# kepingbi/ProdSearch

Measured on AMD Instinct MI355X. Metric: train (u,q,i,neg) tuples/sec at bs=384, 20 neg, d=128, higher is better.
Workload: dtype f32 (fp32 MFMA and VALU; wide products, the fused per-replica kernels and grouped weight gradients as fp32-grade bf16x3 products: exact 3-way bf16 split of both fp32 operands, 6 of the 9 cross products as bf16 MFMAs per step, fp32 accumulation); 1 GPU; item_transformer d=128 1 layer 8 heads ff=512 uprev=20 bs=384/GPU 20 neg Q=8 W=1 P=18357 V=32387 dropout=0.10 (BASELINE configs[1]); global_batch=384, parallelism=dp1, step=sample+fwd+bwd+clip/Adam via nn.Module API (trainer.py:74-78), replicas_per_row=21

## Files before the change

### include/prodsearch_hip.h

```cpp
#ifndef PRODSEARCH_HIP_H
#define PRODSEARCH_HIP_H

#include <stddef.h>
#include <stdint.h>

#ifdef __cplusplus
extern "C" {
#endif

#define PS_MAX_LAYERS 8
#define PS_OK 0
#define PS_ERR_ARG 1
#define PS_ERR_HIP 2

typedef void* ps_stream_t;

enum { PS_MODEL_TEM = 0, PS_MODEL_QEM = 1,
       PS_MODEL_AEM = 2,
       PS_MODEL_ZAM = 3 };
enum { PS_QENC_FS = 0, PS_QENC_AVG = 1 };

typedef struct PsTemDesc {
  int32_t B;
  int32_t K;
// ... 45 lines not shown

typedef struct PsTemBatch {
  const int64_t *query_word_idxs;
  const int64_t *target_prod_idxs;
  const int64_t *u_item_idxs;
  const int64_t *pos_iword_idxs;
  const int64_t *neg_item_idxs;
  const int64_t *neg_word_idxs;
  const int64_t *candi_prod_idxs;
} PsTemBatch;

typedef struct PsTemWsLayout {
  int64_t total_floats;
  int32_t R;
  int32_t S;
  int64_t qmean, query_emb, x;
  int64_t kp, vp, qp, attn, ctx;
  int64_t y1, ln1, a1, h1, y2, enc;
  int64_t item_scores, word_scores, loss_parts;
  int64_t denc, dx;
} PsTemWsLayout;

const char* ps_version(void);
const char* ps_last_error(void);
const char* ps_arith_info(void);
int ps_set_fuse_bwd_min(int rows);
int ps_set_item_scatter_fused(int on);
int ps_item_scatter_fused_taken(void);
typedef struct PsEncPath {
  int32_t n_layers;
  int32_t attn[PS_MAX_LAYERS];
  int32_t rowlist, fwd_fuse_last, fold_score;
  int32_t bwd_fuse_last, item_scatter, wg3_main, wg3_last, wgrad_early, q_folded, listed, presum, dx_fused;
  int32_t wf_key_split;
} PsEncPath;
int ps_tem_plan(const PsTemDesc* desc, const PsTemTensors* params, int32_t has_valid, PsEncPath* out);
int ps_enc_path_taken(int32_t backward, PsEncPath* out);
int ps_set_side_mode(int mode);
int ps_side_values_in_use(void);
void ps_side_abort(void);
void ps_debug_fail_fork(int nth);
int ps_set_deterministic(int on);
int ps_gemm_x3_config(int mode, int force_shape);
int ps_gemm_f32_weight(const float* A, int lda, const float* W, int tb, float* C, int ldc, int M, int N, int K,
                       const float* bias, float alpha, ps_stream_t stream);

int ps_tem_workspace_layout(const PsTemDesc* desc, PsTemWsLayout* out);

int ps_tem_forward(const PsTemDesc* desc, const PsTemTensors* params, const PsTemBatch* batch,
                   float* workspace, float* loss3, float* loss_acc, ps_stream_t stream);
int ps_tem_forward_sampled(const PsTemDesc* desc, const PsTemTensors* params, const PsTemBatch* batch,
                           const float* alias_prob, const int32_t* alias_idx, int64_t* neg_item_out, int64_t* neg_word_out,
                           float* workspace, float* loss3, float* loss_acc, ps_stream_t stream);

int ps_tem_backward(const PsTemDesc* desc, const PsTemTensors* params, const PsTemBatch* batch,
                    float* workspace, const PsTemTensors* grads, float loss_scale,
                    const float* loss_scale_dev ,
                    ps_stream_t stream);

int ps_gather_score(const PsTemDesc* desc, const PsTemTensors* params, const PsTemBatch* batch,
                    float* workspace, ps_stream_t stream);

int ps_tem_score(const PsTemDesc* desc, const PsTemTensors* params, const PsTemBatch* batch,
                 float* workspace, float* scores, ps_stream_t stream);

int ps_sample_negatives(const PsTemDesc* desc, const float* alias_prob, const int32_t* alias_idx,
                        int64_t* neg_item_idxs, int64_t* neg_word_idxs, ps_stream_t stream);
int ps_build_alias_host(const double* dist_host, int64_t n, float* prob_host, int32_t* alias_host);

typedef struct PsAdamHyper {
  float lr;
  float beta1, beta2;
  float eps;
  float weight_decay;
  float max_grad_norm;
  int32_t noam;
  int32_t warmup_steps;
  float grad_scale;
  int32_t zero_grads;
  int32_t method;
  int32_t pad_;
} PsAdamHyper;

int64_t ps_adam_plan_bytes(int32_t n_tensors, const int64_t* numel_host);
int ps_adam_plan_write_host(int32_t n_tensors, float* const* p, float* const* g, float* const* m,
                            float* const* v, const int64_t* numel_host, void* plan_host);
int32_t ps_adam_plan_chunks_host(const void* plan_host);
int ps_clip_adam_dense(const void* plan_dev, int32_t n_chunks, const PsAdamHyper* hyper,
                       int64_t* state_dev, float* gnorm_out_dev ,
                       ps_stream_t stream);

int ps_adam_sumsq(const void* plan_dev, int32_t n_chunks, const PsAdamHyper* hyper, int64_t* state_dev,
                  float* out_sumsq_dev, ps_stream_t stream);
int ps_adam_update_ext(const void* plan_dev, int32_t n_chunks, const PsAdamHyper* hyper, int64_t* state_dev,
                       const float* total_sumsq_dev, float* gnorm_out_dev, ps_stream_t stream);

int ps_sum_slices(const float* recv, int32_t world, int64_t n, float* out, float* zero, int64_t zero_n, ps_stream_t stream);

int ps_zero_floats(float* p, int64_t n, ps_stream_t stream);

int ps_graph_replay_enabled(void);
int ps_tem_staged_batch(const PsTemDesc* desc, float* workspace, PsTemBatch* out);
int ps_tem_forward_step(const PsTemDesc* desc, const PsTemTensors* params, const PsTemBatch* batch,
                        const float* sampler_prob, const int32_t* sampler_alias, float* workspace, float* loss3,
                        float* loss_acc, ps_stream_t stream);
int ps_tem_backward_step(const PsTemDesc* desc, const PsTemTensors* params, float* workspace, const PsTemTensors* grads,
                         float loss_scale, float* zero_ptr, int64_t zero_floats, ps_stream_t stream);

int ps_tem_encode(const PsTemDesc* desc, const PsTemTensors* params, const PsTemBatch* batch, float* workspace,
                  float* enc_out , ps_stream_t stream);
int64_t ps_rank_scratch_bytes(int32_t B, int64_t n_rows, int32_t d, int32_t topk);
int ps_rank_all(const float* q, int32_t B, int32_t d, const float* table, int64_t n_rows, const float* bias,
                const int64_t* target, int32_t topk, int64_t* top_idx, float* top_score, int32_t* rank,
                void* scratch, int64_t scratch_bytes, ps_stream_t stream);
int ps_rank_shard(const float* q, int32_t B, int32_t d, const float* table, int64_t n_rows, const float* bias,
                  const int64_t* target, const float* target_score, int64_t id_mul, int64_t id_add, int32_t topk,
                  int64_t* top_idx, float* top_score, int32_t* ahead, void* scratch, int64_t scratch_bytes, ps_stream_t stream);

typedef struct PsIdxList { const int64_t* idx; int64_t n; } PsIdxList;

int64_t ps_coalesce_ws_bytes(int64_t n_rows);
int ps_coalesce_rows(const PsIdxList* lists_host, int32_t n_lists, int64_t n_rows, int64_t pad_row, void* ws_dev,
                     int64_t* rows_out_dev, int64_t cap, int32_t* count_out_dev, ps_stream_t stream);
int ps_gather_rows(const float* table_dev, int32_t d, const int64_t* rows_dev, const int32_t* count_dev, int64_t cap,
                   float* values_out_dev, ps_stream_t stream);
int ps_scatter_rows(float* table_dev, int32_t d, const int64_t* rows_dev, const int32_t* count_dev, int64_t cap,
                    const float* values_dev, ps_stream_t stream);
int ps_zero_rows(float* table_dev, int32_t d, const int64_t* rows_dev, const int32_t* count_dev, int64_t cap,
                 ps_stream_t stream);
const int32_t* ps_coalesce_bad_flag(void* ws_dev, int64_t n_rows);

int ps_pack_rows(const float* grad_dev, int32_t d, const int64_t* rows_dev, const int32_t* count_dev, int64_t cap,
                 int64_t* msg_rows_dev, float* msg_vals_dev, ps_stream_t stream);
int ps_merge_rows(const int64_t* all_rows_dev, const float* all_vals_dev, int32_t world, int64_t cap, int32_t d,
                  float* grad_dev, const int64_t* union_rows_dev, const int32_t* union_count_dev, int64_t union_cap,
                  ps_stream_t stream);

typedef struct PsRowTable {
  float* p; float* g; float* m; float* v;
  const int64_t* rows;
  const int32_t* count;
  int64_t cap;
  int32_t d;
  int32_t pad_;
} PsRowTable;

int64_t ps_adam_rowsparse_state_floats(int32_t n_chunks, const PsRowTable* tables_host, int32_t n_tables);
int ps_clip_adam_rowsparse(const void* plan_dev, int32_t n_chunks, const PsRowTable* tables_host, int32_t n_tables,
                           const PsAdamHyper* hyper, int64_t* state_dev, float* gnorm_out_dev, ps_stream_t stream);

int ps_rowsparse_catchup(const PsRowTable* tables_host, int32_t n_tables, int32_t* const* last_dev, const int64_t* n_rows_host,
                         const PsAdamHyper* hyper, const int64_t* state_dev, int32_t advance, int32_t all_rows,
                         ps_stream_t stream);

int ps_shard_bucket(const int64_t* rows_dev, const int32_t* count_dev, int32_t world, int64_t capp, int64_t* send_ids_dev,
                    int32_t* slot_of_dev, int32_t* bad_dev, ps_stream_t stream);
int ps_shard_remap(const int64_t* idx_dev, int64_t n, int64_t pad_in, const int64_t* rows_dev, const int32_t* count_dev,
                   const int32_t* slot_of_dev, int64_t pad_out, int64_t* out_dev, int32_t* bad_dev, ps_stream_t stream);
int ps_rowsparse_sumsq(const void* plan_dev, int32_t n_chunks, const PsRowTable* tables_host, int32_t n_tables, int32_t n_shared,
                       const PsAdamHyper* hyper, int64_t* state_dev, float* sums_dev, ps_stream_t stream);
int ps_rowsparse_update_ext(const void* plan_dev, int32_t n_chunks, const PsRowTable* tables_host, int32_t n_tables,
                            const PsAdamHyper* hyper, int64_t* state_dev, const float* sums_dev, float* gnorm_out_dev,
                            ps_stream_t stream);

enum { PS_RENC_PV = 0, PS_RENC_PVC = 1,
       PS_RENC_FS = 2,
// ... 103 lines not shown
```

### prodsearch_amd/_lib.py

```python
import ctypes as C
import os

from . import build as _build

PS_MAX_LAYERS = 8
PS_MODEL_TEM, PS_MODEL_QEM, PS_MODEL_AEM, PS_MODEL_ZAM = 0, 1, 2, 3
PS_QENC_FS, PS_QENC_AVG = 0, 1

_f32p = C.POINTER(C.c_float)
_i64p = C.POINTER(C.c_int64)


class PsTemDesc(C.Structure):
    _fields_ = [(n, C.c_int32) for n in ('B', 'K', 'L', 'Q', 'W', 'C', 'd', 'H', 'F', 'n_layers')] + \
               [('product_size', C.c_int64), ('vocab_size', C.c_int64)] + \
               [(n, C.c_int32) for n in ('model', 'query_encoder', 'use_pos_emb', 'use_item_pos',
                                         'bias_product', 'pos_weight', 'sep_prod_emb', 'training')] + \
               [('dropout', C.c_float), ('seed', C.c_uint64), ('step', C.c_uint64)]


LAYER_FIELDS = ('wk', 'bk', 'wv', 'bv', 'wq', 'bq', 'wo', 'bo', 'w1', 'b1', 'w2', 'b2',
                'ff_ln_g', 'ff_ln_b', 'ln_g', 'ln_b')
TOP_FIELDS = ('product_emb', 'hist_product_emb', 'word_emb', 'product_bias', 'word_bias',
              'fs_w', 'fs_b', 'pe', 'final_ln_g', 'final_ln_b')
# ... 40 lines not shown
class PsRowTable(C.Structure):
    _fields_ = [('p', C.c_void_p), ('g', C.c_void_p), ('m', C.c_void_p), ('v', C.c_void_p),
                ('rows', C.c_void_p), ('count', C.c_void_p), ('cap', C.c_int64), ('d', C.c_int32),
                ('pad_', C.c_int32)]


class PsRtmDesc(C.Structure):
    _fields_ = [(n, C.c_int32) for n in ('B', 'K', 'R', 'Q', 'W', 'WL', 'C', 'd', 'H', 'F', 'n_layers')] + \
               [('vocab_size', C.c_int64), ('review_count', C.c_int64)] + \
               [(n, C.c_int32) for n in ('review_encoder', 'query_encoder', 'use_pos_emb', 'use_seg_emb',
                                         'pos_weight', 'train_pv', 'training')] + \
               [('dropout', C.c_float), ('corrupt_rate', C.c_float), ('seed', C.c_uint64), ('step', C.c_uint64)] + \
               [('use_user_emb', C.c_int32), ('use_item_emb', C.c_int32), ('user_size', C.c_int64),
                ('product_size', C.c_int64)]


RTM_TOP_FIELDS = ('word_emb', 'review_emb', 'seg_emb', 'fs_w', 'fs_b', 'pe', 'final_ln_g', 'final_ln_b',
                  'wo_w', 'wo_b', 'user_emb', 'product_emb', 'rev_fs_w', 'rev_fs_b')
RTM_BATCH_FIELDS = ('query_word_idxs', 'pos_prod_ridxs', 'pos_seg_idxs', 'pos_prod_rword_idxs',
                    'pos_prod_rword_masks', 'neg_prod_ridxs', 'neg_seg_idxs', 'neg_prod_rword_idxs',
                    'pos_prod_rword_idxs_pvc', 'neg_prod_rword_idxs_pvc', 'neg_word_idxs',
                    'candi_prod_ridxs', 'candi_seg_idxs', 'review_embeddings', 'pos_user_idxs', 'neg_user_idxs',
                    'pos_item_idxs', 'neg_item_idxs', 'candi_seq_user_idxs', 'candi_seq_item_idxs', 'neg_prod_rword_masks')


class PsRtmTensors(C.Structure):
    _fields_ = [(n, C.c_void_p) for n in RTM_TOP_FIELDS] + [('layer', PsLayerTensors * PS_MAX_LAYERS)]


class PsRtmBatch(C.Structure):
    _fields_ = [(n, C.c_void_p) for n in RTM_BATCH_FIELDS]


class PsRtmWsLayout(C.Structure):
    _fields_ = [('total_floats', C.c_int64)] + [(n, C.c_int32) for n in ('Bseq', 'S', 'J', 'pad_')] + \
               [(n, C.c_int64) for n in ('query_emb', 'valid', 'x', 'vec', 'cnt', 'enc', 'scores', 'weight',
                                         'pv_scores', 'dx')]


PS_RENC_PV, PS_RENC_PVC, PS_RENC_FS, PS_RENC_AVG = 0, 1, 2, 3

SYMBOLS = {
    'ps_version': (C.c_char_p, []),
    'ps_last_error': (C.c_char_p, []),
    'ps_arith_info': (C.c_char_p, []),
    'ps_set_fuse_bwd_min': (C.c_int, [C.c_int]),
    'ps_set_item_scatter_fused': (C.c_int, [C.c_int]),
    'ps_item_scatter_fused_taken': (C.c_int, []),
    'ps_tem_plan': (C.c_int, [C.POINTER(PsTemDesc), C.POINTER(PsTemTensors), C.c_int32, C.POINTER(PsEncPath)]),
    'ps_enc_path_taken': (C.c_int, [C.c_int32, C.POINTER(PsEncPath)]),
    'ps_set_side_mode': (C.c_int, [C.c_int]),
    'ps_side_values_in_use': (C.c_int, []),
    'ps_set_deterministic': (C.c_int, [C.c_int]),
    'ps_side_abort': (None, []),
    'ps_debug_fail_fork': (None, [C.c_int]),
    'ps_gemm_x3_config': (C.c_int, [C.c_int, C.c_int]),
    'ps_gemm_f32_weight': (C.c_int, [C.c_void_p, C.c_int, C.c_void_p, C.c_int, C.c_void_p, C.c_int, C.c_int, C.c_int, C.c_int,
                                     C.c_void_p, C.c_float, C.c_void_p]),
    'ps_tem_workspace_layout': (C.c_int, [C.POINTER(PsTemDesc), C.POINTER(PsTemWsLayout)]),
    'ps_tem_forward': (C.c_int, [C.POINTER(PsTemDesc), C.POINTER(PsTemTensors), C.POINTER(PsTemBatch),
                                 C.c_void_p, C.c_void_p, C.c_void_p, C.c_void_p]),
    'ps_tem_forward_sampled': (C.c_int, [C.POINTER(PsTemDesc), C.POINTER(PsTemTensors), C.POINTER(PsTemBatch),
                                         C.c_void_p, C.c_void_p, C.c_void_p, C.c_void_p, C.c_void_p, C.c_void_p, C.c_void_p,
                                         C.c_void_p]),
    'ps_tem_backward': (C.c_int, [C.POINTER(PsTemDesc), C.POINTER(PsTemTensors), C.POINTER(PsTemBatch),
                                  C.c_void_p, C.POINTER(PsTemTensors), C.c_float, C.c_void_p, C.c_void_p]),
    'ps_gather_score': (C.c_int, [C.POINTER(PsTemDesc), C.POINTER(PsTemTensors), C.POINTER(PsTemBatch),
                                  C.c_void_p, C.c_void_p]),
    'ps_tem_score': (C.c_int, [C.POINTER(PsTemDesc), C.POINTER(PsTemTensors), C.POINTER(PsTemBatch),
                               C.c_void_p, C.c_void_p, C.c_void_p]),
    'ps_rtm_workspace_floats': (C.c_int, [C.POINTER(PsRtmDesc), C.c_int32, C.POINTER(C.c_int64)]),
    'ps_rtm_workspace_layout': (C.c_int, [C.POINTER(PsRtmDesc), C.c_int32, C.POINTER(PsRtmWsLayout)]),
    'ps_rtm_forward': (C.c_int, [C.POINTER(PsRtmDesc), C.POINTER(PsRtmTensors), C.POINTER(PsRtmBatch),
                                 C.c_void_p, C.c_void_p, C.c_void_p]),
    'ps_rtm_backward': (C.c_int, [C.POINTER(PsRtmDesc), C.POINTER(PsRtmTensors), C.POINTER(PsRtmBatch),
                                  C.c_void_p, C.POINTER(PsRtmTensors), C.c_float, C.c_void_p, C.c_void_p]),
    'ps_rtm_score': (C.c_int, [C.POINTER(PsRtmDesc), C.POINTER(PsRtmTensors), C.POINTER(PsRtmBatch),
                               C.c_void_p, C.c_void_p, C.c_void_p]),
    'ps_rtm_review_embeddings': (C.c_int, [C.POINTER(PsRtmDesc), C.POINTER(PsRtmTensors), C.c_void_p,
                                           C.c_void_p, C.c_void_p, C.c_void_p]),
    'ps_sample_negatives': (C.c_int, [C.POINTER(PsTemDesc), C.c_void_p, C.c_void_p, C.c_void_p,
                                      C.c_void_p, C.c_void_p]),
    'ps_build_alias_host': (C.c_int, [C.c_void_p, C.c_int64, C.c_void_p, C.c_void_p]),
    'ps_adam_plan_bytes': (C.c_int64, [C.c_int32, C.c_void_p]),
    'ps_adam_plan_write_host': (C.c_int, [C.c_int32, C.c_void_p, C.c_void_p, C.c_void_p, C.c_void_p,
                                          C.c_void_p, C.c_void_p]),
    'ps_adam_plan_chunks_host': (C.c_int32, [C.c_void_p]),
    'ps_clip_adam_dense': (C.c_int, [C.c_void_p, C.c_int32, C.POINTER(PsAdamHyper), C.c_void_p,
                                     C.c_void_p, C.c_void_p]),
    'ps_adam_sumsq': (C.c_int, [C.c_void_p, C.c_int32, C.POINTER(PsAdamHyper), C.c_void_p, C.c_void_p, C.c_void_p]),
    'ps_adam_update_ext': (C.c_int, [C.c_void_p, C.c_int32, C.POINTER(PsAdamHyper), C.c_void_p, C.c_void_p, C.c_void_p,
                                     C.c_void_p]),
    'ps_dropout_mult_host': (C.c_float, [C.POINTER(PsTemDesc), C.c_uint32, C.c_uint32, C.c_uint32]),
    'ps_zero_floats': (C.c_int, [C.c_void_p, C.c_int64, C.c_void_p]),
    'ps_sum_slices': (C.c_int, [C.c_void_p, C.c_int32, C.c_int64, C.c_void_p, C.c_void_p, C.c_int64, C.c_void_p]),
    'ps_graph_replay_enabled': (C.c_int, []),
    'ps_tem_staged_batch': (C.c_int, [C.POINTER(PsTemDesc), C.c_void_p, C.POINTER(PsTemBatch)]),
    'ps_tem_forward_step': (C.c_int, [C.POINTER(PsTemDesc), C.POINTER(PsTemTensors), C.POINTER(PsTemBatch), C.c_void_p,
                                      C.c_void_p, C.c_void_p, C.c_void_p, C.c_void_p, C.c_void_p]),
    'ps_tem_backward_step': (C.c_int, [C.POINTER(PsTemDesc), C.POINTER(PsTemTensors), C.c_void_p, C.POINTER(PsTemTensors),
                                       C.c_float, C.c_void_p, C.c_int64, C.c_void_p]),
    'ps_tem_encode': (C.c_int, [C.POINTER(PsTemDesc), C.POINTER(PsTemTensors), C.POINTER(PsTemBatch),
                                C.c_void_p, C.c_void_p, C.c_void_p]),
    'ps_rank_scratch_bytes': (C.c_int64, [C.c_int32, C.c_int64, C.c_int32, C.c_int32]),
    'ps_rank_all': (C.c_int, [C.c_void_p, C.c_int32, C.c_int32, C.c_void_p, C.c_int64, C.c_void_p, C.c_void_p, C.c_int32,
                              C.c_void_p, C.c_void_p, C.c_void_p, C.c_void_p, C.c_int64, C.c_void_p]),
    'ps_rank_shard': (C.c_int, [C.c_void_p, C.c_int32, C.c_int32, C.c_void_p, C.c_int64, C.c_void_p, C.c_void_p, C.c_void_p,
                                C.c_int64, C.c_int64, C.c_int32, C.c_void_p, C.c_void_p, C.c_void_p, C.c_void_p, C.c_int64,
                                C.c_void_p]),
    'ps_coalesce_ws_bytes': (C.c_int64, [C.c_int64]),
    'ps_coalesce_rows': (C.c_int, [C.POINTER(PsIdxList), C.c_int32, C.c_int64, C.c_int64, C.c_void_p,
                                   C.c_void_p, C.c_int64, C.c_void_p, C.c_void_p]),
    'ps_gather_rows': (C.c_int, [C.c_void_p, C.c_int32, C.c_void_p, C.c_void_p, C.c_int64, C.c_void_p, C.c_void_p]),
    'ps_scatter_rows': (C.c_int, [C.c_void_p, C.c_int32, C.c_void_p, C.c_void_p, C.c_int64, C.c_void_p, C.c_void_p]),
    'ps_zero_rows': (C.c_int, [C.c_void_p, C.c_int32, C.c_void_p, C.c_void_p, C.c_int64, C.c_void_p]),
    'ps_coalesce_bad_flag': (C.c_void_p, [C.c_void_p, C.c_int64]),
    'ps_pack_rows': (C.c_int, [C.c_void_p, C.c_int32, C.c_void_p, C.c_void_p, C.c_int64, C.c_void_p, C.c_void_p,
                               C.c_void_p]),
    'ps_merge_rows': (C.c_int, [C.c_void_p, C.c_void_p, C.c_int32, C.c_int64, C.c_int32, C.c_void_p, C.c_void_p,
                                C.c_void_p, C.c_int64, C.c_void_p]),
    'ps_adam_rowsparse_state_floats': (C.c_int64, [C.c_int32, C.POINTER(PsRowTable), C.c_int32]),
    'ps_clip_adam_rowsparse': (C.c_int, [C.c_void_p, C.c_int32, C.POINTER(PsRowTable), C.c_int32,
                                         C.POINTER(PsAdamHyper), C.c_void_p, C.c_void_p, C.c_void_p]),
    'ps_shard_bucket': (C.c_int, [C.c_void_p, C.c_void_p, C.c_int32, C.c_int64, C.c_void_p, C.c_void_p, C.c_void_p, C.c_void_p]),
    'ps_shard_remap': (C.c_int, [C.c_void_p, C.c_int64, C.c_int64, C.c_void_p, C.c_void_p, C.c_void_p, C.c_int64, C.c_void_p,
                                 C.c_void_p, C.c_void_p]),
    'ps_rowsparse_sumsq': (C.c_int, [C.c_void_p, C.c_int32, C.POINTER(PsRowTable), C.c_int32, C.c_int32, C.POINTER(PsAdamHyper),
                                     C.c_void_p, C.c_void_p, C.c_void_p]),
    'ps_rowsparse_update_ext': (C.c_int, [C.c_void_p, C.c_int32, C.POINTER(PsRowTable), C.c_int32, C.POINTER(PsAdamHyper),
                                          C.c_void_p, C.c_void_p, C.c_void_p, C.c_void_p]),
    'ps_rowsparse_catchup': (C.c_int, [C.POINTER(PsRowTable), C.c_int32, C.POINTER(C.c_void_p), C.POINTER(C.c_int64),
                                       C.POINTER(PsAdamHyper), C.c_void_p, C.c_int32, C.c_int32, C.c_void_p]),
    'ps_ktimer_arm': (C.c_int, [C.c_char_p, C.c_int32]),
    'ps_ktimer_read': (C.c_int, [C.POINTER(C.c_double), C.POINTER(C.c_double), C.POINTER(C.c_int32)]),
    'ps_gemm_f32': (C.c_int, [C.c_void_p, C.c_int, C.c_int, C.c_void_p, C.c_int, C.c_int, C.c_void_p,
                              C.c_int, C.c_int, C.c_int, C.c_int, C.c_void_p, C.c_float, C.c_int,
                              C.c_void_p]),
}

class PsCorpusView(C.Structure):
    _fields_ = [(n, C.c_int64) for n in ('n_reviews', 'n_users', 'n_products', 'n_queries')] + \
               [(n, C.c_void_p) for n in ('review_u_p', 'u_seq_ptr', 'u_seq', 'train_review', 'review_loc',
                                          'pq_ptr', 'pq_idx', 'query_words')] + \
               [('Q', C.c_int32), ('pad_', C.c_int32)]


class PsCollateArgs(C.Structure):
    _fields_ = [('uprev_review_limit', C.c_int32), ('do_seq', C.c_int32), ('fix', C.c_int32), ('pad_', C.c_int32),
                ('prod_pad', C.c_int64)]


class PsTrainSlot(C.Structure):
    _fields_ = [(n, C.c_void_p) for n in ('query_words', 'target', 'u_items', 'pos_words', 'query_idx', 'user_idx', 'hist_len')]


class PsRtmCorpusView(C.Structure):
    _fields_ = [(n, C.c_int64) for n in ('n_reviews', 'n_users', 'n_products', 'n_queries')] + \
               [(n, C.c_void_p) for n in ('review_u_p', 'u_seq_ptr', 'u_seq', 'i_seq_ptr', 'i_seq', 'ut_seq_ptr', 'ut_seq',
                                          'it_seq_ptr', 'it_seq', 'loc_time', 'pq_ptr', 'pq_idx', 'query_words')] + \
               [('Q', C.c_int32), ('pad_', C.c_int32)]


class PsRtmCollateArgs(C.Structure):
    _fields_ = [('uprev_review_limit', C.c_int32), ('iprev_review_limit', C.c_int32), ('do_seq', C.c_int32),
                ('neg_per_pos', C.c_int32), ('user_pad', C.c_int64), ('prod_pad', C.c_int64), ('review_pad', C.c_int64)]

# ... 88 lines not shown
```

### prodsearch_amd/csrc/optim.hip

```cpp
#include "optim_core.h"
#include <string.h>

static inline int64_t align16(int64_t x) { return (x + 15) & ~(int64_t)15; }

extern "C" int64_t ps_adam_plan_bytes(int32_t n, const int64_t* numel) {
  int64_t chunks = 0;
  for (int i = 0; i < n; ++i) chunks += (numel[i] + ADAM_CHUNK - 1) / ADAM_CHUNK;
  return align16(sizeof(AdamPlanHeader)) + align16((int64_t)sizeof(AdamChunkRec) * chunks) + 4 * align16(8 * (int64_t)n) +
         align16(8 * (int64_t)n) + align16(4 * (int64_t)(n + 1)) + align16(4 * chunks) + 8 * (int64_t)ADAM_MASK_WORDS * chunks;
}

extern "C" int ps_adam_plan_write_host(int32_t n, float* const* p, float* const* g, float* const* m,
                                       float* const* v, const int64_t* numel, void* plan_host) {
  PS_REQUIRE(n > 0, "adam plan: no tensors");
  char* base = (char*)plan_host;
  AdamPlanHeader h;
  int64_t total_chunks = 0;
  for (int i = 0; i < n; ++i) total_chunks += (numel[i] + ADAM_CHUNK - 1) / ADAM_CHUNK;
  int64_t off = ADAM_REC_OFF + align16((int64_t)sizeof(AdamChunkRec) * total_chunks);
  AdamChunkRec* recs = (AdamChunkRec*)(base + ADAM_REC_OFF);
  h.off_p = off; off += align16(8 * (int64_t)n);
  h.off_g = off; off += align16(8 * (int64_t)n);
  h.off_m = off; off += align16(8 * (int64_t)n);
  h.off_v = off; off += align16(8 * (int64_t)n);
  h.off_numel = off; off += align16(8 * (int64_t)n);
  h.off_chunk0 = off; off += align16(4 * (int64_t)(n + 1));
  h.off_chunk_tensor = off; off += align16(4 * total_chunks);
  h.off_mask = off;
  int32_t* chunk0 = (int32_t*)(base + h.off_chunk0);
  int32_t* chunk_tensor = (int32_t*)(base + h.off_chunk_tensor);
  int64_t chunks = 0;
  for (int i = 0; i < n; ++i) {
    PS_REQUIRE(p[i] && g[i] && m[i] && v[i] && numel[i] > 0, "adam plan: tensor %d null/empty", i);
    ((float**)(base + h.off_p))[i] = p[i];
    ((float**)(base + h.off_g))[i] = g[i];
    ((float**)(base + h.off_m))[i] = m[i];
    ((float**)(base + h.off_v))[i] = v[i];
    ((int64_t*)(base + h.off_numel))[i] = numel[i];
    chunk0[i] = (int32_t)chunks;
    const int64_t nc = (numel[i] + ADAM_CHUNK - 1) / ADAM_CHUNK;
    PS_REQUIRE(chunks + nc < (1 << 30), "adam plan: too many chunks");
    for (int64_t c = 0; c < nc; ++c) {
      chunk_tensor[chunks + c] = i;
      const int64_t beg = c * ADAM_CHUNK, left = numel[i] - beg;
      AdamChunkRec& r = recs[chunks + c];
      r.p = p[i] + beg; r.g = g[i] + beg; r.m = m[i] + beg; r.v = v[i] + beg;
      r.n = (int32_t)(left < ADAM_CHUNK ? left : ADAM_CHUNK); r.pad_ = 0;
    }
    chunks += nc;
  }
  chunk0[n] = (int32_t)chunks;
  PS_REQUIRE(chunks < (1 << 30), "adam plan: too many chunks");
  h.n_tensors = n; h.n_chunks = (int32_t)chunks;
  memcpy(base, &h, sizeof(h));
  return PS_OK;
}

__global__ __launch_bounds__(256) void adam_sumsq_kernel(const char* plan, float grad_scale, int64_t* state,
                                                         float* partial) {
  __shared__ float sh[4];
  const int chunk = blockIdx.x;
  const float s = adam_sumsq_chunk(plan, chunk, grad_scale, sh);
  if (threadIdx.x == 0) {
    partial[chunk] = s;
    if (chunk == 0) state[0] += 1;
  }
}

__global__ __launch_bounds__(256) void adam_update_kernel(const char* plan, const PsAdamHyper hp, const int64_t* state,
                                                          const float* partial, float* gnorm_out) {
  __shared__ float sh[4];
  __shared__ float scal[4];
  const AdamPlanHeader* h = (const AdamPlanHeader*)plan;
  const int chunk = blockIdx.x;
  const float s = strided_sum_f32<8>(partial, h->n_chunks, threadIdx.x, 256);
  const float total = block_sum_256(s, sh);
  if (threadIdx.x == 0) {
    float norm;
    adam_scalars(hp, total, state[0], scal, &norm);
    if (chunk == 0 && gnorm_out) { gnorm_out[0] = norm; gnorm_out[1] = scal[3]; }
  }
  __syncthreads();
  const AdamScal a = {scal[0], scal[1], scal[2], hp.beta1, hp.beta2, hp.eps, hp.weight_decay, hp.zero_grads, scal[3], hp.method};
  adam_update_chunk(plan, chunk, a);
}

extern "C" int ps_clip_adam_dense(const void* plan_dev, int32_t n_chunks, const PsAdamHyper* hyper,
                                    int64_t* state_dev, float* gnorm_out_dev, ps_stream_t stream) {
  PS_REQUIRE(plan_dev && hyper && state_dev && n_chunks > 0, "clip_adam: bad argument");
  PS_REQUIRE(hyper->method >= 0 && hyper->method <= 3, "clip_adam: unknown method %d", hyper->method);
  hipStream_t st = (hipStream_t)stream;
  float* partial = (float*)(state_dev + 2);
  const float gs = hyper->grad_scale == 0.f ? 1.f : hyper->grad_scale;
  PsAdamHyper hp = *hyper;
  hp.grad_scale = gs;
  hipLaunchKernelGGL(adam_sumsq_kernel, dim3(n_chunks), dim3(256), 0, st, (const char*)plan_dev, gs, state_dev,
                     partial);
  PS_LAUNCH_CHECK();
  hipLaunchKernelGGL(adam_update_kernel, dim3(n_chunks), dim3(256), 0, st, (const char*)plan_dev, hp, state_dev,
                     partial, gnorm_out_dev);
  PS_LAUNCH_CHECK();
  return PS_OK;
}

__global__ __launch_bounds__(256) void adam_total_kernel(const float* partial, int n_chunks, float* out) {
  __shared__ float sh[4];
  const float s = strided_sum_f32<8>(partial, n_chunks, threadIdx.x, 256);
  const float total = block_sum_256(s, sh);
  if (threadIdx.x == 0) out[0] = total;
}
__global__ __launch_bounds__(256) void adam_update_ext_kernel(const char* plan, const PsAdamHyper hp, const int64_t* state,
                                                              const float* total_sumsq, float* gnorm_out) {
  __shared__ float scal[4];
  const int chunk = blockIdx.x;
  if (threadIdx.x == 0) {
    float norm;
    adam_scalars(hp, *total_sumsq, state[0], scal, &norm);
    if (chunk == 0 && gnorm_out) { gnorm_out[0] = norm; gnorm_out[1] = scal[3]; }
  }
  __syncthreads();
  const AdamScal a = {scal[0], scal[1], scal[2], hp.beta1, hp.beta2, hp.eps, hp.weight_decay, hp.zero_grads, scal[3], hp.method};
  adam_update_chunk(plan, chunk, a);
}
extern "C" int ps_adam_sumsq(const void* plan_dev, int32_t n_chunks, const PsAdamHyper* hyper, int64_t* state_dev,
                             float* out_sumsq_dev, ps_stream_t stream) {
  PS_REQUIRE(plan_dev && hyper && state_dev && out_sumsq_dev && n_chunks > 0, "adam_sumsq: bad argument");
  hipStream_t st = (hipStream_t)stream;
  float* partial = (float*)(state_dev + 2);
  const float gs = hyper->grad_scale == 0.f ? 1.f : hyper->grad_scale;
  hipLaunchKernelGGL(adam_sumsq_kernel, dim3(n_chunks), dim3(256), 0, st, (const char*)plan_dev, gs, state_dev, partial);
  PS_LAUNCH_CHECK();
  hipLaunchKernelGGL(adam_total_kernel, dim3(1), dim3(256), 0, st, partial, n_chunks, out_sumsq_dev);
  PS_LAUNCH_CHECK();
  return PS_OK;
}
extern "C" int ps_adam_update_ext(const void* plan_dev, int32_t n_chunks, const PsAdamHyper* hyper, int64_t* state_dev,
                                  const float* total_sumsq_dev, float* gnorm_out_dev, ps_stream_t stream) {
  PS_REQUIRE(plan_dev && hyper && state_dev && total_sumsq_dev && n_chunks > 0, "adam_update_ext: bad argument");
  PS_REQUIRE(hyper->method >= 0 && hyper->method <= 3, "adam_update_ext: unknown method %d", hyper->method);
  PsAdamHyper hp = *hyper;
  if (hp.grad_scale == 0.f) hp.grad_scale = 1.f;
  hipLaunchKernelGGL(adam_update_ext_kernel, dim3(n_chunks), dim3(256), 0, (hipStream_t)stream, (const char*)plan_dev, hp,
                     state_dev, total_sumsq_dev, gnorm_out_dev);
  PS_LAUNCH_CHECK();
  return PS_OK;
}

extern "C" int32_t ps_adam_plan_chunks_host(const void* plan_host) {
  return ((const AdamPlanHeader*)plan_host)->n_chunks;
}

__global__ __launch_bounds__(256) void sum_slices_kernel(const float4* __restrict__ recv, int W, int64_t n4, float4* __restrict__ out,
                                                         float4* __restrict__ zero, int64_t zero4) {
  const int64_t stride = (int64_t)gridDim.x * 256;
  for (int64_t i = (int64_t)blockIdx.x * 256 + threadIdx.x; i < n4; i += stride) {
    float4 s = recv[i];
    for (int r = 1; r < W; ++r) {
      const float4 v = recv[(int64_t)r * n4 + i];
      s.x += v.x; s.y += v.y; s.z += v.z; s.w += v.w;
    }
    out[i] = s;
  }
  const float4 z = make_float4(0.f, 0.f, 0.f, 0.f);
  for (int64_t i = (int64_t)blockIdx.x * 256 + threadIdx.x; i < zero4; i += stride) zero[i] = z;
}
extern "C" int ps_sum_slices(const float* recv, int32_t world, int64_t n, float* out, float* zero, int64_t zero_n,
                             ps_stream_t stream) {
  PS_REQUIRE(recv && out && world >= 1 && n >= 0 && n % 4 == 0 && zero_n >= 0 && zero_n % 4 == 0 && (zero || zero_n == 0),
             "sum_slices: bad argument (n %lld, zero_n %lld)", (long long)n, (long long)zero_n);
  PS_REQUIRE((((uintptr_t)recv | (uintptr_t)out | (uintptr_t)zero) & 15) == 0, "sum_slices: buffers must be 16-byte aligned");
  const int64_t work = (n > zero_n ? n : zero_n) / 4;
  if (work == 0) return PS_OK;
  const int grid = (int)(work / 256 + 1 < 2048 ? work / 256 + 1 : 2048);
  hipLaunchKernelGGL(sum_slices_kernel, dim3(grid), dim3(256), 0, (hipStream_t)stream, (const float4*)recv, world, n / 4, (float4*)out,
                     (float4*)zero, zero_n / 4);
  PS_LAUNCH_CHECK();
  return PS_OK;
}

extern "C" int ps_zero_floats(float* p, int64_t n, ps_stream_t stream) {
  PS_REQUIRE(p && n >= 0, "zero: bad argument");
  PS_CHECK_HIP(hipMemsetAsync(p, 0, (size_t)n * sizeof(float), (hipStream_t)stream));
  return PS_OK;
}
```

### prodsearch_amd/csrc/optim_core.h

```cpp
#pragma once
#include "common.h"
#include <math.h>

#define ADAM_CHUNK 4096

struct AdamPlanHeader {
  int32_t n_tensors;
  int32_t n_chunks;
  int64_t off_p, off_g, off_m, off_v, off_numel, off_chunk0;
  int64_t off_chunk_tensor;
  int64_t off_mask;
};
#define ADAM_MASK_WORDS (ADAM_CHUNK / 4 / 64)
struct AdamChunkRec { float* p; float* g; float* m; float* v; int32_t n; int32_t pad_; };
#define ADAM_REC_OFF ((int64_t)((sizeof(AdamPlanHeader) + 15) & ~(size_t)15))
__host__ __device__ inline const AdamChunkRec* adam_chunk_recs(const char* plan) {
  return reinterpret_cast<const AdamChunkRec*>(plan + ADAM_REC_OFF);
}

__device__ inline int find_tensor(const char* plan, const AdamPlanHeader* h, int chunk) {
  return ((const int32_t*)(plan + h->off_chunk_tensor))[chunk];
}

__device__ inline float block_sum_256(float v, float* sh) {
  v = wave_sum(v);
  if ((threadIdx.x & 63) == 0) sh[threadIdx.x >> 6] = v;
  __syncthreads();
  float r = sh[0] + sh[1] + sh[2] + sh[3];
  __syncthreads();
  return r;
}


__device__ inline unsigned long long* adam_chunk_mask(const char* plan, int chunk) {
  return (unsigned long long*)(const_cast<char*>(plan) + ((const AdamPlanHeader*)plan)->off_mask) + (int64_t)chunk * ADAM_MASK_WORDS;
}
__device__ inline float adam_sumsq_chunk(const char* plan, int chunk, float grad_scale, float* sh) {
  const AdamChunkRec rec = adam_chunk_recs(plan)[chunk];
  const float* g = rec.g;
  const int64_t beg = 0, end = rec.n;
  float s = 0.f;
  if ((((uintptr_t)g) & 15) == 0 && end - beg == ADAM_CHUNK) {
    const float4* g4 = (const float4*)(g + beg);
    unsigned long long* mask = adam_chunk_mask(plan, chunk) + (threadIdx.x >> 6) * (ADAM_CHUNK / 4 / 256);
#pragma unroll
    for (int i = 0; i < ADAM_CHUNK / 4 / 256; ++i) {
      float4 x = g4[threadIdx.x + 256 * i];
      const unsigned long long nz = __ballot(x.x != 0.f || x.y != 0.f || x.z != 0.f || x.w != 0.f);
      if ((threadIdx.x & 63) == 0) mask[i] = nz;
      x.x *= grad_scale; x.y *= grad_scale; x.z *= grad_scale; x.w *= grad_scale;
      s += x.x * x.x + x.y * x.y + x.z * x.z + x.w * x.w;
    }
  } else {
    for (int64_t i = beg + threadIdx.x; i < end; i += 256) { float x = g[i] * grad_scale; s += x * x; }
  }
  return block_sum_256(s, sh);
}

__device__ inline void adam_step_scalars(const PsAdamHyper& hp, int64_t step, float* step_size, float* inv_sbc2, float* lr_out) {
  const double t = (double)step;
  double lr = (double)hp.lr;
  if (hp.noam) lr = (double)hp.lr * fmin(pow(t, -0.5), t * pow((double)hp.warmup_steps, -1.5));
  const double bc1 = 1.0 - pow((double)hp.beta1, t);
  const double bc2 = 1.0 - pow((double)hp.beta2, t);
  *step_size = (float)(lr / bc1);
  *inv_sbc2 = (float)(1.0 / sqrt(bc2));
  *lr_out = (float)lr;
}
__device__ inline void adam_scalars(const PsAdamHyper& hp, float total_sumsq, int64_t step, float* out, float* norm_out) {
  const float norm = sqrtf(total_sumsq);
  float coef = 1.f;
  if (hp.max_grad_norm > 0.f) {
    const float c = hp.max_grad_norm / (norm + 1e-6f);
    coef = c >= 1.f ? 1.f : c;
  }
  out[0] = coef * hp.grad_scale;
  adam_step_scalars(hp, step, &out[1], &out[2], &out[3]);
  *norm_out = norm;
}

struct AdamScal { float gmul, step_size, inv_sbc2, b1, b2, eps, wd; int zero_g; float lr; int method; };
#define PS_OPT_ADAM 0
#define PS_OPT_SGD 1
#define PS_OPT_ADAGRAD 2
#define PS_OPT_ADADELTA 3

__device__ inline void adam_elem(const AdamScal& a, float& pp, float gg, float& mm, float& vv) {
#pragma clang fp contract(off)
  gg *= a.gmul;
  if (a.wd != 0.f) gg = __builtin_fmaf(a.wd, pp, gg);
  mm = __builtin_fmaf(gg - mm, 1.f - a.b1, mm);
  vv = vv * a.b2 + ((1.f - a.b2) * gg) * gg;
  const float denom = sqrtf(vv) * a.inv_sbc2 + a.eps;
  pp = pp - a.step_size * (mm / denom);
}

__device__ inline void other_elem(const AdamScal& a, float& pp, float gg, float& s1, float& s2) {
#pragma clang fp contract(off)
  gg *= a.gmul;
  if (a.wd != 0.f) gg = __builtin_fmaf(a.wd, pp, gg);
  if (a.method == PS_OPT_SGD) {
    pp = pp - a.lr * gg;
  } else if (a.method == PS_OPT_ADAGRAD) {
    s1 = __builtin_fmaf(gg, gg, s1);
    pp = pp - a.lr * (gg / (sqrtf(s1) + 1e-10f));
  } else {
    s1 = s1 * 0.9f + (0.1f * gg) * gg;
    const float dlt = (sqrtf(s2 + 1e-6f) / sqrtf(s1 + 1e-6f)) * gg;
    s2 = s2 * 0.9f + (0.1f * dlt) * dlt;
    pp = pp - a.lr * dlt;
  }
}
__device__ inline void other_update_chunk(const AdamChunkRec& rec, const AdamScal& a) {
  float* p = rec.p; float* g = rec.g; float* m = rec.m; float* v = rec.v;
  const bool s1 = a.method != PS_OPT_SGD, s2 = a.method == PS_OPT_ADADELTA;
  for (int i = threadIdx.x; i < rec.n; i += 256) {
    float pp = p[i], gg = g[i], a1 = s1 ? m[i] : 0.f, a2 = s2 ? v[i] : 0.f;
    other_elem(a, pp, gg, a1, a2);
    p[i] = pp;
    if (s1) m[i] = a1;
    if (s2) v[i] = a2;
    if (a.zero_g && gg != 0.f) g[i] = 0.f;
  }
}

__device__ inline void adam_update_chunk(const char* plan, int chunk, const AdamScal& a) {
  const AdamChunkRec rec = adam_chunk_recs(plan)[chunk];
  if (a.method != PS_OPT_ADAM) { other_update_chunk(rec, a); return; }
  float* p = rec.p; float* g = rec.g; float* m = rec.m; float* v = rec.v;
  const int64_t beg = 0, end = rec.n;
  const bool vec = ((((uintptr_t)p) | ((uintptr_t)g) | ((uintptr_t)m) | ((uintptr_t)v)) & 15) == 0 &&
                   end - beg == ADAM_CHUNK;
  if (vec) {
    float4* p4 = (float4*)(p + beg); float4* g4 = (float4*)(g + beg);
    float4* m4 = (float4*)(m + beg); float4* v4 = (float4*)(v + beg);
    const unsigned long long* mask = adam_chunk_mask(plan, chunk) + (threadIdx.x >> 6) * (ADAM_CHUNK / 4 / 256);
    const int lane = threadIdx.x & 63;
#pragma unroll 2
    for (int i = 0; i < ADAM_CHUNK / 4 / 256; ++i) {
      const int k = threadIdx.x + 256 * i;
      const bool nz = (mask[i] >> lane) & 1;
      float4 pp = p4[k], mm = m4[k], vv = v4[k];
      float4 gg = make_float4(0.f, 0.f, 0.f, 0.f);
      if (nz) gg = g4[k];
      if (a.zero_g && nz) g4[k] = make_float4(0.f, 0.f, 0.f, 0.f);
      adam_elem(a, pp.x, gg.x, mm.x, vv.x); adam_elem(a, pp.y, gg.y, mm.y, vv.y);
      adam_elem(a, pp.z, gg.z, mm.z, vv.z); adam_elem(a, pp.w, gg.w, mm.w, vv.w);
      p4[k] = pp; m4[k] = mm; v4[k] = vv;
    }
  } else {
    for (int64_t i = beg + threadIdx.x; i < end; i += 256) {
      float pp = p[i], mm = m[i], vv = v[i];
      adam_elem(a, pp, g[i], mm, vv);
      p[i] = pp; m[i] = mm; v[i] = vv;
      if (a.zero_g && g[i] != 0.f) g[i] = 0.f;
    }
  }
}
```

Measured before the change: 36.36 million tuples/s.

## Restructure Adam update to prefetch params and overlap partial-sum reduction

Step-dependent Adam scalars are now computed once in the sumsq kernel and stored in the plan. The update kernel splits each chunk across two blocks and issues the p/m/v/g loads before reducing the per-chunk squared-norm partials, so the global norm reduction overlaps the memory traffic. Gradient loads for masked-out lanes are redirected to a shared address and zeroed afterwards. The new path is on by default behind PS_ADAM_FORM; it adds diagnostic timestamp hooks and raises register pressure from holding every vector in flight.

After: 37.05 million tuples/s (median of 5 runs). About the same (+1.9%).

```diff
diff --git a/include/prodsearch_hip.h b/include/prodsearch_hip.h
--- a/include/prodsearch_hip.h
+++ b/include/prodsearch_hip.h
@@ -151,6 +151,7 @@
   int32_t pad_;
 } PsAdamHyper;
 
+int ps_set_adam_form(int form);
 int64_t ps_adam_plan_bytes(int32_t n_tensors, const int64_t* numel_host);
 int ps_adam_plan_write_host(int32_t n_tensors, float* const* p, float* const* g, float* const* m,
                             float* const* v, const int64_t* numel_host, void* plan_host);
diff --git a/prodsearch_amd/_lib.py b/prodsearch_amd/_lib.py
--- a/prodsearch_amd/_lib.py
+++ b/prodsearch_amd/_lib.py
@@ -146,6 +146,7 @@
     'ps_sample_negatives': (C.c_int, [C.POINTER(PsTemDesc), C.c_void_p, C.c_void_p, C.c_void_p,
                                       C.c_void_p, C.c_void_p]),
     'ps_build_alias_host': (C.c_int, [C.c_void_p, C.c_int64, C.c_void_p, C.c_void_p]),
+    'ps_set_adam_form': (C.c_int, [C.c_int]),
     'ps_adam_plan_bytes': (C.c_int64, [C.c_int32, C.c_void_p]),
     'ps_adam_plan_write_host': (C.c_int, [C.c_int32, C.c_void_p, C.c_void_p, C.c_void_p, C.c_void_p,
                                           C.c_void_p, C.c_void_p]),
diff --git a/prodsearch_amd/csrc/optim.hip b/prodsearch_amd/csrc/optim.hip
--- a/prodsearch_amd/csrc/optim.hip
+++ b/prodsearch_amd/csrc/optim.hip
@@ -1,5 +1,9 @@
 #include "optim_core.h"
 #include <string.h>
+#include <utility>
+
+static int& adam_form_slot() { static int v = ps_env_int("PS_ADAM_FORM", 1); return v; }
+extern "C" int ps_set_adam_form(int form) { return form < 0 ? adam_form_slot() : std::exchange(adam_form_slot(), form); }
 
 static inline int64_t align16(int64_t x) { return (x + 15) & ~(int64_t)15; }
 
@@ -7,7 +11,7 @@
   int64_t chunks = 0;
   for (int i = 0; i < n; ++i) chunks += (numel[i] + ADAM_CHUNK - 1) / ADAM_CHUNK;
   return align16(sizeof(AdamPlanHeader)) + align16((int64_t)sizeof(AdamChunkRec) * chunks) + 4 * align16(8 * (int64_t)n) +
-         align16(8 * (int64_t)n) + align16(4 * (int64_t)(n + 1)) + align16(4 * chunks) + 8 * (int64_t)ADAM_MASK_WORDS * chunks;
+         align16(8 * (int64_t)n) + align16(4 * (int64_t)(n + 1)) + align16(4 * chunks) + 8 * (int64_t)ADAM_MASK_WORDS * chunks + 16;
 }
 
 extern "C" int ps_adam_plan_write_host(int32_t n, float* const* p, float* const* g, float* const* m,
@@ -26,7 +30,8 @@
   h.off_numel = off; off += align16(8 * (int64_t)n);
   h.off_chunk0 = off; off += align16(4 * (int64_t)(n + 1));
   h.off_chunk_tensor = off; off += align16(4 * total_chunks);
-  h.off_mask = off;
+  h.off_mask = off; off += 8 * (int64_t)ADAM_MASK_WORDS * total_chunks;
+  h.off_scal = off;
   int32_t* chunk0 = (int32_t*)(base + h.off_chunk0);
   int32_t* chunk_tensor = (int32_t*)(base + h.off_chunk_tensor);
   int64_t chunks = 0;
@@ -56,8 +61,8 @@
   return PS_OK;
 }
 
-__global__ __launch_bounds__(256) void adam_sumsq_kernel(const char* plan, float grad_scale, int64_t* state,
-                                                         float* partial) {
+__global__ __launch_bounds__(256) void adam_sumsq_form0_kernel(const char* plan, float grad_scale, int64_t* state,
+                                                               float* partial) {
   __shared__ float sh[4];
   const int chunk = blockIdx.x;
   const float s = adam_sumsq_chunk(plan, chunk, grad_scale, sh);
@@ -67,10 +72,17 @@
   }
 }
 
-__global__ __launch_bounds__(256) void adam_update_kernel(const char* plan, const PsAdamHyper hp, const int64_t* state,
-                                                          const float* partial, float* gnorm_out) {
+__global__ __launch_bounds__(256) void adam_update_form0_kernel(const char* plan, const PsAdamHyper hp, const int64_t* state,
+                                                                const float* partial, float* gnorm_out, unsigned long long* stamp) {
   __shared__ float sh[4];
   __shared__ float scal[4];
+#if PS_DIAG_ON
+  unsigned long long tkbuf[6] = {0, 0, 0, 0, 0, 0};
+  unsigned long long* tk = stamp ? tkbuf : nullptr;
+#else
+  unsigned long long* tk = nullptr;
+#endif
+  ADAM_STAMP(tk, 0);
   const AdamPlanHeader* h = (const AdamPlanHeader*)plan;
   const int chunk = blockIdx.x;
   const float s = strided_sum_f32<8>(partial, h->n_chunks, threadIdx.x, 256);
@@ -82,8 +94,30 @@
   }
   __syncthreads();
   const AdamScal a = {scal[0], scal[1], scal[2], hp.beta1, hp.beta2, hp.eps, hp.weight_decay, hp.zero_grads, scal[3], hp.method};
-  adam_update_chunk(plan, chunk, a);
-}
+  ADAM_STAMP(tk, 1);
+  adam_update_chunk(plan, chunk, a, tk);
+  ADAM_STAMP_END(tk, stamp);
+}
+
+__global__ __launch_bounds__(256) void adam_sumsq_kernel(const char* plan, const PsAdamHyper hp, int64_t* state, float* partial) {
+  __shared__ float sh[4];
+  const int chunk = blockIdx.x;
+  if (chunk == 0 && threadIdx.x == 0) {
+    const int64_t step = state[0] + 1;
+    state[0] = step;
+    float* sc = (float*)(const_cast<char*>(plan) + ((const AdamPlanHeader*)plan)->off_scal);
+    adam_step_scalars(hp, step, &sc[0], &sc[1], &sc[2]);
+  }
+  const float s = adam_sumsq_chunk(plan, chunk, hp.grad_scale, sh);
+  if (threadIdx.x == 0) partial[chunk] = s;
+}
+
+__global__ __launch_bounds__(256) void adam_update_kernel(const char* plan, const PsAdamHyper hp, const float* partial,
+                                                          int n_chunks, float* gnorm_out, unsigned long long* stamp) {
+  adam_update_front<false>(plan, hp, partial, n_chunks, gnorm_out, stamp);
+}
+
+static unsigned long long* adam_stamp_ptr() { return ps_diag_int("PS_ADAM_STAMP", 0) ? ps_debug_stamp_ptr() : nullptr; }
 
 extern "C" int ps_clip_adam_dense(const void* plan_dev, int32_t n_chunks, const PsAdamHyper* hyper,
                                     int64_t* state_dev, float* gnorm_out_dev, ps_stream_t stream) {
@@ -94,12 +128,23 @@
   const float gs = hyper->grad_scale == 0.f ? 1.f : hyper->grad_scale;
   PsAdamHyper hp = *hyper;
   hp.grad_scale = gs;
-  hipLaunchKernelGGL(adam_sumsq_kernel, dim3(n_chunks), dim3(256), 0, st, (const char*)plan_dev, gs, state_dev,
-                     partial);
-  PS_LAUNCH_CHECK();
-  hipLaunchKernelGGL(adam_update_kernel, dim3(n_chunks), dim3(256), 0, st, (const char*)plan_dev, hp, state_dev,
-                     partial, gnorm_out_dev);
-  PS_LAUNCH_CHECK();
+  const bool front = adam_form_slot() != 0;
+  {
+    KTimeScope kt("adam_sumsq", st);
+    if (front) PS_KLAUNCH(adam_sumsq_kernel, dim3(n_chunks), dim3(256), 0, st, (const char*)plan_dev, hp, state_dev, partial);
+    else PS_KLAUNCH(adam_sumsq_form0_kernel, dim3(n_chunks), dim3(256), 0, st, (const char*)plan_dev, gs, state_dev, partial);
+    PS_LAUNCH_CHECK();
+  }
+  {
+    KTimeScope kt("adam_update", st);
+    if (front)
+      PS_KLAUNCH(adam_update_kernel, dim3(ADAM_FRONT_NB * n_chunks), dim3(256), 0, st, (const char*)plan_dev, hp, (const float*)partial,
+                 n_chunks, gnorm_out_dev, adam_stamp_ptr());
+    else
+      PS_KLAUNCH(adam_update_form0_kernel, dim3(n_chunks), dim3(256), 0, st, (const char*)plan_dev, hp, (const int64_t*)state_dev,
+                 (const float*)partial, gnorm_out_dev, adam_stamp_ptr());
+    PS_LAUNCH_CHECK();
+  }
   return PS_OK;
 }
 
@@ -109,8 +154,8 @@
   const float total = block_sum_256(s, sh);
   if (threadIdx.x == 0) out[0] = total;
 }
-__global__ __launch_bounds__(256) void adam_update_ext_kernel(const char* plan, const PsAdamHyper hp, const int64_t* state,
-                                                              const float* total_sumsq, float* gnorm_out) {
+__global__ __launch_bounds__(256) void adam_update_ext_form0_kernel(const char* plan, const PsAdamHyper hp, const int64_t* state,
+                                                                    const float* total_sumsq, float* gnorm_out) {
   __shared__ float scal[4];
   const int chunk = blockIdx.x;
   if (threadIdx.x == 0) {
@@ -121,14 +166,22 @@
   __syncthreads();
   const AdamScal a = {scal[0], scal[1], scal[2], hp.beta1, hp.beta2, hp.eps, hp.weight_decay, hp.zero_grads, scal[3], hp.method};
   adam_update_chunk(plan, chunk, a);
+}
+__global__ __launch_bounds__(256) void adam_update_ext_kernel(const char* plan, const PsAdamHyper hp, const float* total_sumsq,
+                                                              float* gnorm_out) {
+  adam_update_front<true>(plan, hp, total_sumsq, 0, gnorm_out, nullptr);
 }
 extern "C" int ps_adam_sumsq(const void* plan_dev, int32_t n_chunks, const PsAdamHyper* hyper, int64_t* state_dev,
                              float* out_sumsq_dev, ps_stream_t stream) {
   PS_REQUIRE(plan_dev && hyper && state_dev && out_sumsq_dev && n_chunks > 0, "adam_sumsq: bad argument");
   hipStream_t st = (hipStream_t)stream;
   float* partial = (float*)(state_dev + 2);
-  const float gs = hyper->grad_scale == 0.f ? 1.f : hyper->grad_scale;
-  hipLaunchKernelGGL(adam_sumsq_kernel, dim3(n_chunks), dim3(256), 0, st, (const char*)plan_dev, gs, state_dev, partial);
+  PsAdamHyper hp = *hyper;
+  if (hp.grad_scale == 0.f) hp.grad_scale = 1.f;
+  if (adam_form_slot() != 0)
+    hipLaunchKernelGGL(adam_sumsq_kernel, dim3(n_chunks), dim3(256), 0, st, (const char*)plan_dev, hp, state_dev, partial);
+  else
+    hipLaunchKernelGGL(adam_sumsq_form0_kernel, dim3(n_chunks), dim3(256), 0, st, (const char*)plan_dev, hp.grad_scale, state_dev, partial);
   PS_LAUNCH_CHECK();
   hipLaunchKernelGGL(adam_total_kernel, dim3(1), dim3(256), 0, st, partial, n_chunks, out_sumsq_dev);
   PS_LAUNCH_CHECK();
@@ -140,8 +193,12 @@
   PS_REQUIRE(hyper->method >= 0 && hyper->method <= 3, "adam_update_ext: unknown method %d", hyper->method);
   PsAdamHyper hp = *hyper;
   if (hp.grad_scale == 0.f) hp.grad_scale = 1.f;
-  hipLaunchKernelGGL(adam_update_ext_kernel, dim3(n_chunks), dim3(256), 0, (hipStream_t)stream, (const char*)plan_dev, hp,
-                     state_dev, total_sumsq_dev, gnorm_out_dev);
+  if (adam_form_slot() != 0)
+    hipLaunchKernelGGL(adam_update_ext_kernel, dim3(ADAM_FRONT_NB * n_chunks), dim3(256), 0, (hipStream_t)stream, (const char*)plan_dev, hp,
+                       total_sumsq_dev, gnorm_out_dev);
+  else
+    hipLaunchKernelGGL(adam_update_ext_form0_kernel, dim3(n_chunks), dim3(256), 0, (hipStream_t)stream, (const char*)plan_dev, hp,
+                       (const int64_t*)state_dev, total_sumsq_dev, gnorm_out_dev);
   PS_LAUNCH_CHECK();
   return PS_OK;
 }
diff --git a/prodsearch_amd/csrc/optim_core.h b/prodsearch_amd/csrc/optim_core.h
--- a/prodsearch_amd/csrc/optim_core.h
+++ b/prodsearch_amd/csrc/optim_core.h
@@ -10,6 +10,7 @@
   int64_t off_p, off_g, off_m, off_v, off_numel, off_chunk0;
   int64_t off_chunk_tensor;
   int64_t off_mask;
+  int64_t off_scal;
 };
 #define ADAM_MASK_WORDS (ADAM_CHUNK / 4 / 64)
 struct AdamChunkRec { float* p; float* g; float* m; float* v; int32_t n; int32_t pad_; };
@@ -67,16 +68,19 @@
   *inv_sbc2 = (float)(1.0 / sqrt(bc2));
   *lr_out = (float)lr;
 }
-__device__ inline void adam_scalars(const PsAdamHyper& hp, float total_sumsq, int64_t step, float* out, float* norm_out) {
+__device__ inline float adam_clip_gmul(const PsAdamHyper& hp, float total_sumsq, float* norm_out) {
   const float norm = sqrtf(total_sumsq);
   float coef = 1.f;
   if (hp.max_grad_norm > 0.f) {
     const float c = hp.max_grad_norm / (norm + 1e-6f);
     coef = c >= 1.f ? 1.f : c;
   }
-  out[0] = coef * hp.grad_scale;
+  *norm_out = norm;
+  return coef * hp.grad_scale;
+}
+__device__ inline void adam_scalars(const PsAdamHyper& hp, float total_sumsq, int64_t step, float* out, float* norm_out) {
+  out[0] = adam_clip_gmul(hp, total_sumsq, norm_out);
   adam_step_scalars(hp, step, &out[1], &out[2], &out[3]);
-  *norm_out = norm;
 }
 
 struct AdamScal { float gmul, step_size, inv_sbc2, b1, b2, eps, wd; int zero_g; float lr; int method; };
@@ -124,7 +128,32 @@
   }
 }
 
-__device__ inline void adam_update_chunk(const char* plan, int chunk, const AdamScal& a) {
+#if PS_DIAG_ON
+#define ADAM_STAMP(tk, slot)                                                                          \
+  do {                                                                                                \
+    if (tk) asm volatile("s_memrealtime %0\n\ts_waitcnt lgkmcnt(0)" : "=s"((tk)[slot])::"memory"); \
+  } while (0)
+#define ADAM_STAMP_ARRIVED(tk, slot, x)                     \
+  do {                                                      \
+    if (tk) { asm volatile("" ::"v"(x)); ADAM_STAMP(tk, slot); } \
+  } while (0)
+#define ADAM_STAMP_END(tk, stamp)                                                            \
+  do {                                                                                       \
+    if (tk) {                                                                                \
+      ADAM_STAMP(tk, 4);                                                                     \
+      asm volatile("s_waitcnt vmcnt(0)" ::: "memory");                                       \
+      ADAM_STAMP(tk, 5);                                                                     \
+      if (threadIdx.x == 0)                                                                  \
+        for (int k_ = 0; k_ < 6; ++k_) (stamp)[8 * (int64_t)blockIdx.x + k_] = (tk)[k_];    \
+    }                                                                                        \
+  } while (0)
+#else
+#define ADAM_STAMP_END(tk, stamp) do { } while (0)
+#define ADAM_STAMP(tk, slot) do { } while (0)
+#define ADAM_STAMP_ARRIVED(tk, slot, x) do { } while (0)
+#endif
+
+__device__ inline void adam_update_chunk(const char* plan, int chunk, const AdamScal& a, unsigned long long* tk = nullptr) {
   const AdamChunkRec rec = adam_chunk_recs(plan)[chunk];
   if (a.method != PS_OPT_ADAM) { other_update_chunk(rec, a); return; }
   float* p = rec.p; float* g = rec.g; float* m = rec.m; float* v = rec.v;
@@ -141,8 +170,10 @@
       const int k = threadIdx.x + 256 * i;
       const bool nz = (mask[i] >> lane) & 1;
       float4 pp = p4[k], mm = m4[k], vv = v4[k];
+      if (i == 0) ADAM_STAMP_ARRIVED(tk, 2, vv.w);
       float4 gg = make_float4(0.f, 0.f, 0.f, 0.f);
       if (nz) gg = g4[k];
+      if (i == 0) ADAM_STAMP_ARRIVED(tk, 3, gg.w);
       if (a.zero_g && nz) g4[k] = make_float4(0.f, 0.f, 0.f, 0.f);
       adam_elem(a, pp.x, gg.x, mm.x, vv.x); adam_elem(a, pp.y, gg.y, mm.y, vv.y);
       adam_elem(a, pp.z, gg.z, mm.z, vv.z); adam_elem(a, pp.w, gg.w, mm.w, vv.w);
@@ -157,3 +188,124 @@
     }
   }
 }
+
+
+typedef float adam_f4 __attribute__((ext_vector_type(4)));
+typedef __attribute__((address_space(1))) adam_f4 adam_gf4;
+__device__ __forceinline__ void adam_elem4(const AdamScal& a, adam_f4& p, adam_f4 g, adam_f4& m, adam_f4& v) {
+  float pe[4] = {p.x, p.y, p.z, p.w}, me[4] = {m.x, m.y, m.z, m.w}, ve[4] = {v.x, v.y, v.z, v.w};
+  const float ge[4] = {g.x, g.y, g.z, g.w};
+#pragma unroll
+  for (int e = 0; e < 4; ++e) adam_elem(a, pe[e], ge[e], me[e], ve[e]);
+  p = (adam_f4){pe[0], pe[1], pe[2], pe[3]}; m = (adam_f4){me[0], me[1], me[2], me[3]}; v = (adam_f4){ve[0], ve[1], ve[2], ve[3]};
+}
+
+__device__ __forceinline__ float adam_partials_thread_sum(const float (&pv)[8], const float* __restrict__ sums, int n, int tid) {
+  float s = 0.f;
+#pragma unroll
+  for (int u = 0; u < 8; ++u) s = __builtin_fmaf(pv[u], tid + 256 * u < n ? 1.f : 0.f, s);
+  if (tid >= n) s = 0.f;
+  for (int i = tid + 2048; i < n; i += 2048) {
+    float v[8];
+#pragma unroll
+    for (int u = 0; u < 8; ++u) { const int j = i + 256 * u; v[u] = sums[j < n ? j : 0]; }
+#pragma unroll
+    for (int u = 0; u < 8; ++u) s = __builtin_fmaf(v[u], i + 256 * u < n ? 1.f : 0.f, s);
+  }
+  return s;
+}
+__device__ __forceinline__ float adam_block_total(float s, float* sh) {
+  s = wave_sum(s);
+  if ((threadIdx.x & 63) == 0) sh[threadIdx.x >> 6] = s;
+  __syncthreads();
+  return sh[0] + sh[1] + sh[2] + sh[3];
+}
+
+#define ADAM_FRONT_NB 2
+template <bool EXT>
+__device__ __forceinline__ void adam_update_front(const char* plan, const PsAdamHyper& hp, const float* __restrict__ sums,
+                                                  int n_sums, float* gnorm_out, unsigned long long* stamp) {
+  constexpr int NB = ADAM_FRONT_NB;
+  __shared__ float sh[4];
+  constexpr int IT = ADAM_CHUNK / 4 / 256 / NB;
+  static_assert(IT * NB == 4, "adam_update_front: four mask words per wave of a chunk");
+  const int chunk = blockIdx.x / NB, part = blockIdx.x % NB, tid = threadIdx.x, lane = tid & 63;
+  const int wave = __builtin_amdgcn_readfirstlane(tid >> 6);
+#if PS_DIAG_ON
+  unsigned long long tkbuf[6] = {0, 0, 0, 0, 0, 0};
+  unsigned long long* tk = stamp ? tkbuf : nullptr;
+#else
+  unsigned long long* tk = nullptr;
+#endif
+  ADAM_STAMP(tk, 0);
+  const AdamPlanHeader* h = (const AdamPlanHeader*)plan;
+  const AdamChunkRec rec = adam_chunk_recs(plan)[chunk];
+  const float* sc = (const float*)(plan + h->off_scal);
+  const unsigned long long* mw = (const unsigned long long*)(plan + h->off_mask) + (int64_t)chunk * ADAM_MASK_WORDS + wave * 4;
+  float pv[8];
+  if (!EXT) {
+#pragma unroll
+    for (int u = 0; u < 8; ++u) { const int j = tid + 256 * u; pv[u] = sums[j < n_sums ? j : 0]; }
+  }
+  const float step_size = sc[0], inv_sbc2 = sc[1], lr = sc[2];
+  const bool front = hp.method == PS_OPT_ADAM && rec.n == ADAM_CHUNK &&
+                     ((((uintptr_t)rec.p) | ((uintptr_t)rec.g) | ((uintptr_t)rec.m) | ((uintptr_t)rec.v)) & 15) == 0;
+  if (front) {
+    const int first = part * IT * 256;
+    adam_gf4* p4 = (adam_gf4*)(uintptr_t)rec.p + first; adam_gf4* g4 = (adam_gf4*)(uintptr_t)rec.g + first;
+    adam_gf4* m4 = (adam_gf4*)(uintptr_t)rec.m + first; adam_gf4* v4 = (adam_gf4*)(uintptr_t)rec.v + first;
+    const unsigned long long* mwp = mw + part * IT;
+    unsigned long long wv[IT];
+#pragma unroll
+    for (int i = 0; i < IT; ++i) wv[i] = mwp[i];
+    const unsigned tu = (unsigned)tid;
+    adam_f4 pp[IT], mm[IT], vv[IT], gg[IT];
+#pragma unroll
+    for (int i = 0; i < IT; ++i) { pp[i] = (p4 + 256 * i)[tu]; mm[i] = (m4 + 256 * i)[tu]; vv[i] = (v4 + 256 * i)[tu]; }
+    unsigned long long w[IT];
+#pragma unroll
+    for (int i = 0; i < IT; ++i)
+      w[i] = (unsigned long long)(unsigned)__builtin_amdgcn_readfirstlane((int)(unsigned)wv[i]) |
+             ((unsigned long long)(unsigned)__builtin_amdgcn_readfirstlane((int)(unsigned)(wv[i] >> 32)) << 32);
+    float s = 0.f;
+    if (!EXT) s = adam_partials_thread_sum(pv, sums, n_sums, tid);
+    asm volatile("" ::: "memory");
+#pragma unroll
+    for (int i = 0; i < IT; ++i) gg[i] = (g4 + 256 * i)[((w[i] >> lane) & 1) ? tu : tu - (unsigned)lane];
+    asm volatile("" ::: "memory");
+    const float total = EXT ? sums[0] : adam_block_total(s, sh);
+    float norm;
+    const float gmul = adam_clip_gmul(hp, total, &norm);
+    if (blockIdx.x == 0 && tid == 0 && gnorm_out) { gnorm_out[0] = norm; gnorm_out[1] = lr; }
+    const AdamScal a = {gmul, step_size, inv_sbc2, hp.beta1, hp.beta2, hp.eps, hp.weight_decay, hp.zero_grads, lr, hp.method};
+    ADAM_STAMP(tk, 1);
+    ADAM_STAMP_ARRIVED(tk, 2, vv[0].w);
+    ADAM_STAMP_ARRIVED(tk, 3, gg[IT - 1].w);
+#pragma unroll
+    for (int i = 0; i < IT; ++i) {
+      if (!((w[i] >> lane) & 1)) gg[i] = (adam_f4){0.f, 0.f, 0.f, 0.f};
+      adam_elem4(a, pp[i], gg[i], mm[i], vv[i]);
+    }
+#pragma unroll
+    for (int i = 0; i < IT; ++i) { (p4 + 256 * i)[tu] = pp[i]; (m4 + 256 * i)[tu] = mm[i]; (v4 + 256 * i)[tu] = vv[i]; }
+    if (a.zero_g) {
+#pragma unroll
+      for (int i = 0; i < IT; ++i)
+        if (w[i] != 0) (g4 + 256 * i)[tu] = (adam_f4){0.f, 0.f, 0.f, 0.f};
+    }
+    ADAM_STAMP_END(tk, stamp);
+    return;
+  }
+  if (part != 0) return;
+  {
+    const float total = EXT ? sums[0] : block_sum_256(strided_sum_f32<8>(sums, n_sums, tid, 256), sh);
+    float norm;
+    const float gmul = adam_clip_gmul(hp, total, &norm);
+    if (chunk == 0 && tid == 0 && gnorm_out) { gnorm_out[0] = norm; gnorm_out[1] = lr; }
+    const AdamScal a = {gmul, step_size, inv_sbc2, hp.beta1, hp.beta2, hp.eps, hp.weight_decay, hp.zero_grads, lr, hp.method};
+    ADAM_STAMP(tk, 1);
+    adam_update_chunk(plan, chunk, a, tk);
+  }
+  ADAM_STAMP_END(tk, stamp);
+  __builtin_amdgcn_s_waitcnt(0);
+}
```
